# zhengjingsen/LidarDetection

Measured on AMD Instinct MI355X. Metric: frames/sec (fwd+NMS) PointPillar-KITTI, higher is better.
Workload: dtype f32; 1 GPU; PointPillar-KITTI bs=16 per GPU, fp32, eval BN folded: HIP voxelize + PFN; dense 2D backbone = first layer from the pillars (sparse implicit GEMM), stride-1 3x3 layers as Winograd F(4x4,3x3) on the fp32 MFMA, strided deblocks as one fused MFMA GEMM (all this repo's HIP), the two stride-2 3x3 layers MIOpen, stride-1 deblock + 1x1 heads hipBLASLt; exact HIP top-k + decode + batched rotated NMS; clou; replicas=1

## Files before the change

### lidardetection_amd/csrc/build.py

```python
import glob
import os
import subprocess
import sys

HERE = os.path.dirname(os.path.abspath(__file__))
SO = os.path.join(HERE, "liblidar_hip.so")
HIPCC = os.environ.get("HIPCC", "/opt/rocm/bin/hipcc")
FLAGS = ["--offload-arch=gfx950", "-O3", "-fPIC", "-std=c++17", "-ffp-contract=off", "-fvisibility=hidden",
         "-Wall", "-Wno-unused-function"]
EXTRA_FLAGS = {"wino43_conv.hip": ["-mllvm", "-pragma-unroll-threshold=4000000", "-Wno-inline-asm"]}


def sources():
    return sorted(glob.glob(os.path.join(HERE, "*.hip")))


def build(force=False, verbose=False):
    srcs = sources()
    deps = srcs + glob.glob(os.path.join(HERE, "*.h")) + [os.path.abspath(__file__)]
    if not force and os.path.exists(SO) and all(os.path.getmtime(SO) >= os.path.getmtime(d) for d in deps):
        return SO
    objs = []
    procs = []
    for s in srcs:
        o = s[:-4] + ".o"
        if (not force and os.path.exists(o)
                and all(os.path.getmtime(o) >= os.path.getmtime(d) for d in [s] + deps[len(srcs):])):
            objs.append(o)
            continue
        cmd = [HIPCC, *FLAGS, *EXTRA_FLAGS.get(os.path.basename(s), []), "-c", s, "-o", o]
        if verbose:
            print(" ".join(cmd))
        procs.append((s, subprocess.Popen(cmd)))
        objs.append(o)
    for s, p in procs:
        if p.wait() != 0:
            raise RuntimeError(f"hipcc failed on {s}")
    cmd = [HIPCC, "--offload-arch=gfx950", "-shared", "-fPIC", "-o", SO, *objs]
    if verbose:
        print(" ".join(cmd))
    subprocess.check_call(cmd)
    return SO


VARIANTS = {
    "vxl_nowait": ("voxelize.hip", ["-DVXL_WAIT_TICKS=0"]),
}
AB_VARIANTS = {
    "w43_aux0": ("wino43_conv.hip", ["-DW43_STORE_AUX=0"]),
    "vxl_fill_nt": ("voxelize.hip", ["-DVXL_FILL_NT=1"]),
    "vxl_share12": ("voxelize.hip", ["-DVXL_FILL_SHARE16=12"]), "vxl_share10": ("voxelize.hip", ["-DVXL_FILL_SHARE16=10"]),
    "vxl_share8": ("voxelize.hip", ["-DVXL_FILL_SHARE16=8"]),
    "dc_nowait": ("deconv_gemm.hip", ["-DDC_PROBE=1"]),
    "sc_p1": ("sparse_conv.hip", ["-DSC_PROBE=1"]), "sc_p2": ("sparse_conv.hip", ["-DSC_PROBE=2"]), "sc_p4": ("sparse_conv.hip", ["-DSC_PROBE=4"]),
    "sc_p7": ("sparse_conv.hip", ["-DSC_PROBE=7"]),
}


def variant_path(name):
    return os.path.join(HERE, f"liblidar_hip_{name}.so")


def build_variants(force=False, verbose=False, names=None):
    build(force=False, verbose=verbose)
    outs = []
    todo = VARIANTS if names is None else {n: {**VARIANTS, **AB_VARIANTS}[n] for n in names}
    for name, (src, extra) in todo.items():
        so = variant_path(name)
        s = os.path.join(HERE, src)
        deps = [s] + glob.glob(os.path.join(HERE, "*.h")) + [os.path.abspath(__file__), SO]
        if not force and os.path.exists(so) and all(os.path.getmtime(so) >= os.path.getmtime(d) for d in deps):
            outs.append(so)
            continue
        o = os.path.join(HERE, f"{src[:-4]}.{name}.o")
        cmd = [HIPCC, *FLAGS, *EXTRA_FLAGS.get(src, []), *extra, "-c", s, "-o", o]
        if verbose:
            print(" ".join(cmd))
        subprocess.check_call(cmd)
        objs = [x[:-4] + ".o" for x in sources() if os.path.basename(x) != src] + [o]
        subprocess.check_call([HIPCC, "--offload-arch=gfx950", "-shared", "-fPIC", "-o", so, *objs])
        outs.append(so)
    return outs


if __name__ == "__main__":
    print(build(force="--force" in sys.argv, verbose=True))
    print(build_variants(force="--force" in sys.argv, verbose=True))
```

### lidardetection_amd/csrc/deconv_gemm.hip

```cpp
#include "common.h"
#ifndef DC_PROBE
#define DC_PROBE 0
#endif

typedef float f32x16 __attribute__((ext_vector_type(16)));
typedef float f32x4 __attribute__((ext_vector_type(4)));
typedef unsigned u32x4 __attribute__((ext_vector_type(4)));
typedef float f32x2 __attribute__((ext_vector_type(2)));

#define DC_OOB 0x80000000u

__global__ __launch_bounds__(256) void dc_pack_kernel(const float *__restrict__ W, int K, int N, float *__restrict__ P) {
    const long long idx = (long long)blockIdx.x * 256 + threadIdx.x;
    if (idx >= (long long)K * N) return;
    const int k = (int)(idx / N), col = (int)(idx - (long long)k * N);
    const int c = k >> 2, h = (k >> 1) & 1, s = k & 1, g = col >> 9, t = (col >> 5) & 15, j = col & 31, NG = N >> 9;
    P[(((((size_t)c * NG + g) * 8 + (t >> 1)) * 64 + (h * 32 + j)) * 2 + (t & 1)) * 2 + s] = W[idx];
}

struct DcArgs {
    const float *in;
    const float *pk;
    const float *bias;
    float *out;
    int P, K, N, h, w, s, C_up, out_C, out_off, relu;
    int n_pblocks, n_groups, n_blocks;
    unsigned out_bytes;
};

#define DC_STG_PITCH 132
static constexpr size_t dc_lds_bytes() { return (size_t)2 * 128 * 16 + (size_t)4 * 32 * DC_STG_PITCH * 4; }

__global__ __launch_bounds__(256) void dc_gemm_kernel(const DcArgs a) {
    extern __shared__ float4 s_mem4[];
    float4 *s_a = s_mem4;
    float *s_stg = reinterpret_cast<float *>(s_mem4 + 2 * 128);
    const int t = threadIdx.x, l = t & 63, wv = __builtin_amdgcn_readfirstlane(t >> 6);
    const int i = l & 31, h = l >> 5;
    const int K = a.K, NC = K >> 2;
    const int bstride = a.n_groups * 8 * 64;

    const int nb8 = (a.n_blocks + 7) >> 3;
    const __amdgpu_buffer_rsrc_t orsrc = __builtin_amdgcn_make_buffer_rsrc(a.out, (short)0, (int)a.out_bytes, 0x00020000);
    const int xcd = (int)(blockIdx.x & 7), slot = (int)(blockIdx.x >> 3), nslots = (int)(gridDim.x >> 3);
    const int blk_end = min((xcd + 1) * nb8, a.n_blocks);
    int blk = xcd * nb8 + slot;
    if (blk >= blk_end) return;

    struct Tile {
        unsigned aoff;
        int b;
        int p0, g;
    };
    auto make_tile = [&](int blk_) {
        Tile tl;
        tl.g = blk_ % a.n_groups;
        const int pb = blk_ / a.n_groups;
        tl.p0 = pb * 128;
        const int p = tl.p0 + 64 * (wv & 1) + l;
        tl.aoff = p < a.P ? (unsigned)p * (unsigned)K * 4u : DC_OOB;
        tl.b = tl.g * 8 * 64;
        return tl;
    };
    typedef int i32x4 __attribute__((ext_vector_type(4)));
    i32x4 arsrc;
    {
        const unsigned long long base = (unsigned long long)a.in;
        arsrc[0] = (int)(unsigned)base;
        arsrc[1] = (int)((unsigned)(base >> 32) & 0xffffu);
        arsrc[2] = (int)((unsigned)a.P * (unsigned)K * 4u);
        arsrc[3] = 0x00020000;
    }
    const __amdgpu_buffer_rsrc_t brsrc = __builtin_amdgcn_make_buffer_rsrc(const_cast<float *>(a.pk), (short)0, (int)((unsigned)K * (unsigned)a.N * 4u), 0x00020000);
    const int l16 = l * 16;
    auto ldb = [&](int f4_index) { return __builtin_bit_cast(f32x4, __builtin_amdgcn_raw_buffer_load_b128(brsrc, l16, f4_index * 16, 0)); };
    const unsigned a_lds = (unsigned)(size_t)((__attribute__((address_space(3))) char *)s_a);
    unsigned doff = 0;
    auto dma = [&](int buf) {
        if (wv < 2) {
            const unsigned dst = a_lds + (unsigned)((buf * 128 + 64 * wv) * 16);
            asm volatile("s_mov_b32 m0, %2\n\ts_nop 0\n\tbuffer_load_dwordx4 %0, %1, 0 offen lds" : : "v"(doff), "s"(arsrc), "s"(dst) : "memory", "m0");
        }
    };
    auto load_a = [&](int buf, f32x2 &av) { av = reinterpret_cast<const f32x2 *>(s_a + buf * 128 + 32 * wv + i)[h]; };

    f32x16 acc[16];
    f32x2 a0, a1;
    f32x4 b0[8], b1[8];
    Tile cur = make_tile(blk), nxt = cur;
    doff = cur.aoff;
    dma(0);
    doff += 16u;
    dma(1);
    doff += 16u;
#pragma unroll
    for (int e = 0; e < 8; ++e) b0[e] = ldb(cur.b + e * 64);
    __builtin_amdgcn_s_waitcnt(0x0F70);
    asm volatile("" ::: "memory");
    __syncthreads();
    load_a(0, a0);
    __syncthreads();

#define DC_CHUNK(c, P, FIRST, AC, BC, AN, BN)                                                                                      \
    {                                                                                                                              \
        if ((c) > 0) {                                                                                                             \
            if (DC_PROBE & 1) asm volatile("s_waitcnt lgkmcnt(0)\n\ts_barrier" ::: "memory");                                      \
            else asm volatile("s_waitcnt vmcnt(8) lgkmcnt(0)\n\ts_barrier" ::: "memory");                                          \
        } else if (!first_block) asm volatile("s_waitcnt lgkmcnt(0)\n\ts_barrier" ::: "memory");                                   \
        dma(P);                                                                                        \
        doff = ((c) + 3 == NC) ? (has_next ? nxt.aoff : DC_OOB) : doff + 16u;                                                      \
        const int bn_ = ((c) + 1 < NC) ? cur.b + ((c) + 1) * bstride : (has_next ? nxt.b : cur.b);                                 \
        const f32x2 *as_ = reinterpret_cast<const f32x2 *>(s_a + (1 - (P)) * 128 + 32 * wv + i) + h;                               \
        __builtin_amdgcn_sched_barrier(0);                                                                                         \
        _Pragma("unroll") for (int k = 0; k < 32; ++k) {                                                                           \
            const float bop_ = BC[(k & 15) >> 1][((k & 1) << 1) + (k >> 4)];                                                       \
            if (FIRST && k < 16) {                                                                                                 \
                f32x16 z_;                                                                                                         \
                _Pragma("unroll") for (int r_ = 0; r_ < 16; ++r_) z_[r_] = 0.f;                                                    \
                acc[k & 15] = __builtin_amdgcn_mfma_f32_32x32x2f32(AC[k >> 4], bop_, z_, 0, 0, 0);                                 \
            } else {                                                                                                               \
                acc[k & 15] = __builtin_amdgcn_mfma_f32_32x32x2f32(AC[k >> 4], bop_, acc[k & 15], 0, 0, 0);                        \
            }                                                                                                                      \
            if (k < 8) BN[k] = ldb(bn_ + k * 64);                                                                                  \
            if (k == 2) AN = as_[0];                                                                                               \
            __builtin_amdgcn_sched_barrier(0);                                                                                     \
        }                                                                                                                          \
    }

    bool first_block = true;
    for (;;) {
        const int blk_next = blk + nslots;
        const bool has_next = blk_next < blk_end;
        if (has_next) nxt = make_tile(blk_next);
        DC_CHUNK(0, 0, true, a0, b0, a1, b1)
        DC_CHUNK(1, 1, false, a1, b1, a0, b0)
        for (int c = 2; c < NC; c += 2) {
            DC_CHUNK(c, 0, false, a0, b0, a1, b1)
            DC_CHUNK(c + 1, 1, false, a1, b1, a0, b0)
        }
        {
            __builtin_amdgcn_s_waitcnt(0x0F70);
            int lo = l;
            asm volatile("" : "+v"(lo));
            const bool relu = a.relu != 0;
            float *stg = s_stg + (size_t)wv * 32 * DC_STG_PITCH;
            const int hw = a.h * a.w, OW = a.s * a.w;
            unsigned pix[16];
            {
                const int p = cur.p0 + 32 * wv + (lo >> 5);
                int bb = p / hw;
                const int rem = p - bb * hw;
                int y = rem / a.w, x = rem - y * a.w;
#pragma unroll
                for (int k = 0; k < 16; ++k) {
                    pix[k] = (p + 2 * k < a.P) ? (unsigned)(((bb * a.s * a.h + a.s * y) * OW + a.s * x) * a.out_C + a.out_off + 4 * (lo & 31)) * 4u : 0x80000000u;
#pragma unroll
                    for (int st = 0; st < 2; ++st) {
                        x += 1;
                        if (x >= a.w) { x = 0; y += 1; }
                        if (y >= a.h) { y = 0; bb += 1; }
                    }
                }
            }
#pragma unroll
            for (int rnd = 0; rnd < 4; ++rnd) {
                const int col0 = 512 * cur.g + 128 * rnd;
                const int kk = col0 / a.C_up, c0 = col0 - kk * a.C_up;
                const int ky = kk / a.s, kx = kk - ky * a.s;
#pragma unroll
                for (int nn = 0; nn < 4; ++nn) {
                    const float bvv = a.bias ? a.bias[c0 + 32 * nn + i] : 0.f;
                    float m[16];
#pragma unroll
                    for (int r = 0; r < 16; ++r) asm volatile("v_accvgpr_read_b32 %0, %1" : "=v"(m[r]) : "a"(acc[4 * rnd + nn][r]));
#pragma unroll
                    for (int r = 0; r < 16; ++r) {
                        const int row = 8 * (r >> 2) + 4 * h + (r & 3);
                        const float v = m[r] + bvv;
                        stg[row * DC_STG_PITCH + 32 * nn + i] = relu ? fmaxf(v, 0.f) : v;
                    }
                    __builtin_amdgcn_sched_barrier(0);
                }
                const int soff = ((ky * OW + kx) * a.out_C + c0) * 4;
#pragma unroll
                for (int k4 = 0; k4 < 16; k4 += 4) {
                    f32x4 sv[4];
#pragma unroll
                    for (int k = 0; k < 4; ++k) sv[k] = *reinterpret_cast<const f32x4 *>(stg + (2 * (k4 + k) + (lo >> 5)) * DC_STG_PITCH + 4 * (lo & 31));
#pragma unroll
                    for (int k = 0; k < 4; ++k)
                        __builtin_amdgcn_raw_buffer_store_b128(__builtin_bit_cast(u32x4, sv[k]), orsrc, (int)pix[k4 + k], soff, 0);
                    __builtin_amdgcn_sched_barrier(0);
                }
            }
        }
        if (!has_next) break;
        cur = nxt;
        blk = blk_next;
        first_block = false;
    }
#undef DC_CHUNK
}

LIDAR_EXPORT size_t lidar_deconv_packed_floats(int K, int N) {
    if (K < 16 || N <= 0 || (K & 7) || (N & 511)) return 0;
    return (size_t)K * N;
}

LIDAR_EXPORT int lidar_deconv_supported(int K, int s, int C_up) {
    if (s <= 0 || C_up <= 0 || (C_up & 127)) return 0;
    return lidar_deconv_packed_floats(K, s * s * C_up) != 0;
}

LIDAR_EXPORT int lidar_deconv_pack_weights(const float *W, int K, int N, float *packed, void *stream) {
    if (!W || !packed || lidar_deconv_packed_floats(K, N) == 0) return LIDAR_ERR_ARG;
    hipLaunchKernelGGL(dc_pack_kernel, dim3(divup((long long)K * N, 256)), dim3(256), 0, (hipStream_t)stream, W, K, N, packed);
    return lidar_check_launch("lidar_deconv_pack_weights");
}

static int dc_cu_count() {
    static int cus[64] = {};
    int dev = 0, n = 0;
    if (hipGetDevice(&dev) != hipSuccess) return 256;
    dev &= 63;
    if (cus[dev] == 0) cus[dev] = (hipDeviceGetAttribute(&n, hipDeviceAttributeMultiprocessorCount, dev) == hipSuccess && n > 0) ? n : 256;
    return cus[dev];
}

LIDAR_EXPORT int lidar_deconv_gemm_nhwc(const float *in, int B, int h, int w, int K, const float *packed, const float *bias, int relu, int s,
                                        int C_up, float *out, int out_C, int out_off, void *stream) {
    if (!in || !packed || !out || B <= 0 || h <= 0 || w <= 0 || !lidar_deconv_supported(K, s, C_up) || out_off < 0 || out_off + C_up > out_C)
        return LIDAR_ERR_ARG;
    if ((reinterpret_cast<uintptr_t>(in) & 15) || (reinterpret_cast<uintptr_t>(packed) & 15) || (reinterpret_cast<uintptr_t>(out) & 15) ||
        (out_C & 3) || (out_off & 3) || (long long)B * h * w > 0x7fffffffll || (long long)B * h * w * s * s * out_C * 4 >= 0x7fffffffll ||
        (long long)B * h * w * K * 4 >= 0x7fffffffll || (long long)K * s * s * C_up * 4 >= 0x7fffffffll)
        return LIDAR_ERR_ARG;
    DcArgs a;
    a.in = in; a.pk = packed; a.bias = bias; a.out = out;
    a.P = B * h * w; a.K = K; a.N = s * s * C_up; a.h = h; a.w = w; a.s = s; a.C_up = C_up; a.out_C = out_C; a.out_off = out_off; a.relu = relu;
    a.out_bytes = (unsigned)((long long)B * h * w * s * s * out_C * 4);
    a.n_pblocks = divup(a.P, 128);
    a.n_groups = a.N / 512;
    const long long nblk = (long long)a.n_pblocks * a.n_groups;
    if (nblk > 0x7ffffff0ll) return LIDAR_ERR_ARG;
    a.n_blocks = (int)nblk;
    long long want = ((nblk + 7) / 8) * 8;
    const long long cap = ((long long)dc_cu_count() / 8) * 8;
    if (cap >= 8 && want > cap) want = cap;
    static bool attr_set[64] = {};
    int dev_id = 0;
    (void)hipGetDevice(&dev_id);
    dev_id &= 63;
    if (!attr_set[dev_id]) {
        (void)hipFuncSetAttribute(reinterpret_cast<const void *>(&dc_gemm_kernel), hipFuncAttributeMaxDynamicSharedMemorySize, (int)dc_lds_bytes());
        attr_set[dev_id] = true;
    }
    hipLaunchKernelGGL(dc_gemm_kernel, dim3((unsigned)want), dim3(256), dc_lds_bytes(), (hipStream_t)stream, a);
    return lidar_check_launch("lidar_deconv_gemm_nhwc");
}
```

Baseline: 3307 frames/s.

## Load deconv GEMM A operand directly from global instead of LDS DMA staging

Replaces the double-buffered buffer_load-to-LDS DMA of the A tile, along with the per-chunk barriers and waitcnts, with per-lane 64-bit buffer loads straight into registers. Each load is issued one chunk ahead and prefetches across tiles. This removes the LDS A buffers and the workgroup barriers from the inner loop, at the cost of more, narrower global loads with each wave fetching its own rows. It also adds probe variants that skip the epilogue or the stores for timing.

Measured after the change: 3313 frames/s, median of 6. About the same (+0.2%).

```diff
diff --git a/lidardetection_amd/csrc/build.py b/lidardetection_amd/csrc/build.py
--- a/lidardetection_amd/csrc/build.py
+++ b/lidardetection_amd/csrc/build.py
@@ -51,7 +51,7 @@
     "vxl_fill_nt": ("voxelize.hip", ["-DVXL_FILL_NT=1"]),
     "vxl_share12": ("voxelize.hip", ["-DVXL_FILL_SHARE16=12"]), "vxl_share10": ("voxelize.hip", ["-DVXL_FILL_SHARE16=10"]),
     "vxl_share8": ("voxelize.hip", ["-DVXL_FILL_SHARE16=8"]),
-    "dc_nowait": ("deconv_gemm.hip", ["-DDC_PROBE=1"]),
+    "dc_noepi": ("deconv_gemm.hip", ["-DDC_PROBE=2"]), "dc_nostore": ("deconv_gemm.hip", ["-DDC_PROBE=4"]),
     "sc_p1": ("sparse_conv.hip", ["-DSC_PROBE=1"]), "sc_p2": ("sparse_conv.hip", ["-DSC_PROBE=2"]), "sc_p4": ("sparse_conv.hip", ["-DSC_PROBE=4"]),
     "sc_p7": ("sparse_conv.hip", ["-DSC_PROBE=7"]),
 }
diff --git a/lidardetection_amd/csrc/deconv_gemm.hip b/lidardetection_amd/csrc/deconv_gemm.hip
--- a/lidardetection_amd/csrc/deconv_gemm.hip
+++ b/lidardetection_amd/csrc/deconv_gemm.hip
@@ -29,12 +29,11 @@
 };
 
 #define DC_STG_PITCH 132
-static constexpr size_t dc_lds_bytes() { return (size_t)2 * 128 * 16 + (size_t)4 * 32 * DC_STG_PITCH * 4; }
+static constexpr size_t dc_lds_bytes() { return (size_t)4 * 32 * DC_STG_PITCH * 4; }
 
 __global__ __launch_bounds__(256) void dc_gemm_kernel(const DcArgs a) {
     extern __shared__ float4 s_mem4[];
-    float4 *s_a = s_mem4;
-    float *s_stg = reinterpret_cast<float *>(s_mem4 + 2 * 128);
+    float *s_stg = reinterpret_cast<float *>(s_mem4);
     const int t = threadIdx.x, l = t & 63, wv = __builtin_amdgcn_readfirstlane(t >> 6);
     const int i = l & 31, h = l >> 5;
     const int K = a.K, NC = K >> 2;
@@ -57,60 +56,31 @@
         tl.g = blk_ % a.n_groups;
         const int pb = blk_ / a.n_groups;
         tl.p0 = pb * 128;
-        const int p = tl.p0 + 64 * (wv & 1) + l;
-        tl.aoff = p < a.P ? (unsigned)p * (unsigned)K * 4u : DC_OOB;
+        const int p = tl.p0 + 32 * wv + i;
+        tl.aoff = p < a.P ? (unsigned)p * (unsigned)K * 4u + 8u * (unsigned)h : DC_OOB;
         tl.b = tl.g * 8 * 64;
         return tl;
     };
-    typedef int i32x4 __attribute__((ext_vector_type(4)));
-    i32x4 arsrc;
-    {
-        const unsigned long long base = (unsigned long long)a.in;
-        arsrc[0] = (int)(unsigned)base;
-        arsrc[1] = (int)((unsigned)(base >> 32) & 0xffffu);
-        arsrc[2] = (int)((unsigned)a.P * (unsigned)K * 4u);
-        arsrc[3] = 0x00020000;
-    }
+    const __amdgpu_buffer_rsrc_t arsrc = __builtin_amdgcn_make_buffer_rsrc(const_cast<float *>(a.in), (short)0, (int)((unsigned)a.P * (unsigned)K * 4u), 0x00020000);
     const __amdgpu_buffer_rsrc_t brsrc = __builtin_amdgcn_make_buffer_rsrc(const_cast<float *>(a.pk), (short)0, (int)((unsigned)K * (unsigned)a.N * 4u), 0x00020000);
     const int l16 = l * 16;
     auto ldb = [&](int f4_index) { return __builtin_bit_cast(f32x4, __builtin_amdgcn_raw_buffer_load_b128(brsrc, l16, f4_index * 16, 0)); };
-    const unsigned a_lds = (unsigned)(size_t)((__attribute__((address_space(3))) char *)s_a);
-    unsigned doff = 0;
-    auto dma = [&](int buf) {
-        if (wv < 2) {
-            const unsigned dst = a_lds + (unsigned)((buf * 128 + 64 * wv) * 16);
-            asm volatile("s_mov_b32 m0, %2\n\ts_nop 0\n\tbuffer_load_dwordx4 %0, %1, 0 offen lds" : : "v"(doff), "s"(arsrc), "s"(dst) : "memory", "m0");
-        }
-    };
-    auto load_a = [&](int buf, f32x2 &av) { av = reinterpret_cast<const f32x2 *>(s_a + buf * 128 + 32 * wv + i)[h]; };
+    auto lda = [&](unsigned aoff, int chunk) { return __builtin_bit_cast(f32x2, __builtin_amdgcn_raw_buffer_load_b64(arsrc, (int)aoff, chunk * 16, 0)); };
 
     f32x16 acc[16];
     f32x2 a0, a1;
     f32x4 b0[8], b1[8];
     Tile cur = make_tile(blk), nxt = cur;
-    doff = cur.aoff;
-    dma(0);
-    doff += 16u;
-    dma(1);
-    doff += 16u;
+    a0 = lda(cur.aoff, 0);
+    a1 = lda(cur.aoff, 1);
 #pragma unroll
     for (int e = 0; e < 8; ++e) b0[e] = ldb(cur.b + e * 64);
-    __builtin_amdgcn_s_waitcnt(0x0F70);
-    asm volatile("" ::: "memory");
-    __syncthreads();
-    load_a(0, a0);
-    __syncthreads();
-
-#define DC_CHUNK(c, P, FIRST, AC, BC, AN, BN)                                                                                      \
+
+#define DC_CHUNK(c, FIRST, AC, BC, BN)                                                                                             \
     {                                                                                                                              \
-        if ((c) > 0) {                                                                                                             \
-            if (DC_PROBE & 1) asm volatile("s_waitcnt lgkmcnt(0)\n\ts_barrier" ::: "memory");                                      \
-            else asm volatile("s_waitcnt vmcnt(8) lgkmcnt(0)\n\ts_barrier" ::: "memory");                                          \
-        } else if (!first_block) asm volatile("s_waitcnt lgkmcnt(0)\n\ts_barrier" ::: "memory");                                   \
-        dma(P);                                                                                        \
-        doff = ((c) + 3 == NC) ? (has_next ? nxt.aoff : DC_OOB) : doff + 16u;                                                      \
         const int bn_ = ((c) + 1 < NC) ? cur.b + ((c) + 1) * bstride : (has_next ? nxt.b : cur.b);                                 \
-        const f32x2 *as_ = reinterpret_cast<const f32x2 *>(s_a + (1 - (P)) * 128 + 32 * wv + i) + h;                               \
+        const unsigned ao_ = ((c) + 2 < NC) ? cur.aoff : (has_next ? nxt.aoff : DC_OOB);                                           \
+        const int ac_ = ((c) + 2 < NC) ? (c) + 2 : (c) + 2 - NC;                                                                   \
         __builtin_amdgcn_sched_barrier(0);                                                                                         \
         _Pragma("unroll") for (int k = 0; k < 32; ++k) {                                                                           \
             const float bop_ = BC[(k & 15) >> 1][((k & 1) << 1) + (k >> 4)];                                                       \
@@ -122,24 +92,25 @@
                 acc[k & 15] = __builtin_amdgcn_mfma_f32_32x32x2f32(AC[k >> 4], bop_, acc[k & 15], 0, 0, 0);                        \
             }                                                                                                                      \
             if (k < 8) BN[k] = ldb(bn_ + k * 64);                                                                                  \
-            if (k == 2) AN = as_[0];                                                                                               \
+            if (k == 31) AC = lda(ao_, ac_);                                                                                       \
             __builtin_amdgcn_sched_barrier(0);                                                                                     \
         }                                                                                                                          \
     }
 
-    bool first_block = true;
     for (;;) {
         const int blk_next = blk + nslots;
         const bool has_next = blk_next < blk_end;
         if (has_next) nxt = make_tile(blk_next);
-        DC_CHUNK(0, 0, true, a0, b0, a1, b1)
-        DC_CHUNK(1, 1, false, a1, b1, a0, b0)
+        DC_CHUNK(0, true, a0, b0, b1)
+        DC_CHUNK(1, false, a1, b1, b0)
         for (int c = 2; c < NC; c += 2) {
-            DC_CHUNK(c, 0, false, a0, b0, a1, b1)
-            DC_CHUNK(c + 1, 1, false, a1, b1, a0, b0)
+            DC_CHUNK(c, false, a0, b0, b1)
+            DC_CHUNK(c + 1, false, a1, b1, b0)
         }
-        {
-            __builtin_amdgcn_s_waitcnt(0x0F70);
+        if (DC_PROBE & 2) {
+#pragma unroll
+            for (int n = 0; n < 16; ++n) asm volatile("" : : "a"(acc[n]));
+        } else {
             int lo = l;
             asm volatile("" : "+v"(lo));
             const bool relu = a.relu != 0;
@@ -188,8 +159,10 @@
 #pragma unroll
                     for (int k = 0; k < 4; ++k) sv[k] = *reinterpret_cast<const f32x4 *>(stg + (2 * (k4 + k) + (lo >> 5)) * DC_STG_PITCH + 4 * (lo & 31));
 #pragma unroll
-                    for (int k = 0; k < 4; ++k)
-                        __builtin_amdgcn_raw_buffer_store_b128(__builtin_bit_cast(u32x4, sv[k]), orsrc, (int)pix[k4 + k], soff, 0);
+                    for (int k = 0; k < 4; ++k) {
+                        if (DC_PROBE & 4) asm volatile("" : : "v"(sv[k]), "v"(pix[k4 + k]), "s"(soff));
+                        else __builtin_amdgcn_raw_buffer_store_b128(__builtin_bit_cast(u32x4, sv[k]), orsrc, (int)pix[k4 + k], soff, 0);
+                    }
                     __builtin_amdgcn_sched_barrier(0);
                 }
             }
@@ -197,7 +170,6 @@
         if (!has_next) break;
         cur = nxt;
         blk = blk_next;
-        first_block = false;
     }
 #undef DC_CHUNK
 }
```
